# ZhangXinWhut/SimWhisper-Codec

Hardware: AMD Instinct MI355X
Metric: audio-sec/sec encode+decode (RTF^-1), 16kHz batch=32x10s (higher is better)
Workload: dtype split-f16 x3 encode (f32-class, f32 accumulate) / bf16 decode (f32 accumulate); 1 GPU; batch=32x10s @16kHz per GPU (32 utterances in all), encode()+decode(), 0.1*N(0,1) seed 1234, synthetic closed-form checkpoint (291M params); precision=mixed

## Files before the change

include/swc.h:

```cpp
#ifndef SWC_H_
#define SWC_H_

#include <stdint.h>

#ifdef __cplusplus
extern "C" {
#endif

#define SWC_OK 0
#define SWC_E_ARG (-1)
#define SWC_E_LAUNCH (-2)
#define SWC_E_NODEV (-3)

#define SWC_F32 0
#define SWC_BF16 1
#define SWC_F16S 2
#define SWC_F16S_ACT_SCALE 64.0f
#define SWC_FP8 3
#define SWC_FP8_ACT_SCALE 16.0f
#define SWC_F16 4

#define SWC_ACT_NONE 0
#define SWC_ACT_GELU 1

int swc_version(void);
const char* swc_last_error(void);
int swc_device_count(void);

int swc_delay_us(int32_t us, void* stream);

int swc_set_saturation_counter(uint32_t* counters);

typedef struct swc_gemm_args {
    const void* A;
    const void* W;
    void* C;
    const float* bias;
    const float* gamma;
    const float* residual;
    int64_t lda, ldw, ldc, ldr;
    int32_t M, N, K;
    int32_t taps, dil, stride, pad, t_in, t_out;
    int32_t a_dtype, c_dtype, act;
    float alpha;
    float out_scale;
} swc_gemm_args;
int swc_gemm(const swc_gemm_args* args, void* stream);
typedef struct swc_gemm_plan_out {
    int32_t a_dtype;
    int32_t tile_m, tile_n;
    int32_t waves;
    int32_t plain;
    int32_t act_body;
    int32_t k_slice, k_slices;
    int32_t n_tiles_m, n_tiles_n;
    int32_t band;
    int32_t grid, slots;
} swc_gemm_plan_out;
int swc_gemm_plan(const swc_gemm_args* args, swc_gemm_plan_out* plan);

int swc_attention(const void* qkv, void* out, const int32_t* lens, int32_t B, int32_t T,
                  int32_t H, int32_t dtype, void* stream);
int swc_attention16(const void* qkv, void* out, const int32_t* lens, int32_t B, int32_t T, int32_t H,
                    int32_t dtype, const int32_t* row_start, void* stream);
int swc_attention_ex(const void* qkv, void* out, const int32_t* lens, int32_t B, int32_t T, int32_t H,
                     int32_t out_dtype, void* stream);

int swc_layernorm(const float* x, void* y, const float* w, const float* b, const int32_t* lens,
                  int32_t B, int32_t t_in, int32_t t_out, int32_t C, float eps, int32_t y_dtype,
                  const int32_t* row_start, void* stream);

int swc_pack_rows(const void* src, void* dst, const int32_t* row_start, const int32_t* lens, int32_t B, int32_t T,
                  int64_t row_bytes, void* stream);

int64_t swc_convnext_stream_bytes(int32_t C, int32_t I);
int swc_convnext_pack(const void* w1_16bit, const void* w2_16bit, const float* gamma, void* w_stream, int32_t C, int32_t I,
                      void* stream);
int swc_convnext_mlp(const void* y, const void* w_stream, const float* b1, const float* b2, const float* gamma,
                     float* x, int32_t M, int32_t C, int32_t I, void* stream);
int swc_convnext_block(const float* x, float* x_out, const float* dw_w7, const float* dw_bias, const float* ln_w,
// ... 96 lines not shown
```

simwhisper_codec_amd/_lib.py:

```python
import ctypes as C
import os

import torch

HERE = os.path.dirname(os.path.abspath(__file__))
LIB_PATH = os.environ.get("SWC_LIB") or os.path.join(HERE, "libswc_hip.so")

F32, BF16, F16S, FP8 = 0, 1, 2, 3
F16S_ACT_SCALE = 64.0
FP8_ACT_SCALE = 16.0
ACT_NONE, ACT_GELU = 0, 1


class SwcError(RuntimeError):
    pass


class GemmArgs(C.Structure):
    _fields_ = [
        ("A", C.c_void_p), ("W", C.c_void_p), ("C", C.c_void_p),
        ("bias", C.c_void_p), ("gamma", C.c_void_p), ("residual", C.c_void_p),
        ("lda", C.c_int64), ("ldw", C.c_int64), ("ldc", C.c_int64), ("ldr", C.c_int64),
        ("M", C.c_int32), ("N", C.c_int32), ("K", C.c_int32),
        ("taps", C.c_int32), ("dil", C.c_int32), ("stride", C.c_int32), ("pad", C.c_int32),
        ("t_in", C.c_int32), ("t_out", C.c_int32),
        ("a_dtype", C.c_int32), ("c_dtype", C.c_int32), ("act", C.c_int32),
        ("alpha", C.c_float), ("out_scale", C.c_float),
    ]


class GemmPlan(C.Structure):
    _fields_ = [(n, C.c_int32) for n in ("a_dtype", "tile_m", "tile_n", "waves", "plain", "act_body", "k_slice", "k_slices",
                                         "n_tiles_m", "n_tiles_n", "band", "grid", "slots")]


class Dwconv7LnPlan(C.Structure):
    _fields_ = [(n, C.c_int32) for n in ("S", "NK", "FULL", "nst", "nstrips", "slots", "per", "grid")]


_P, _I, _L, _F = C.c_void_p, C.c_int32, C.c_int64, C.c_float

SIGNATURES = {
    "swc_gemm": [C.POINTER(GemmArgs), _P],
    "swc_gemm_plan": [C.POINTER(GemmArgs), C.POINTER(GemmPlan)],
    "swc_attention": [_P, _P, _P, _I, _I, _I, _I, _P],
    "swc_attention_ex": [_P, _P, _P, _I, _I, _I, _I, _P],
    "swc_attention16": [_P, _P, _P, _I, _I, _I, _I, _P, _P],
    "swc_layernorm": [_P, _P, _P, _P, _P, _I, _I, _I, _I, _F, _I, _P, _P],
    "swc_dwconv7_ln": [_P, _P, _P, _P, _P, _P, _I, _I, _I, _F, _I, _P],
    "swc_dwconv7_ln_plan": [_I, _I, _I, _I, C.POINTER(Dwconv7LnPlan)],
    "swc_snake_aa": [_P, _P, _P, _P, C.POINTER(_F), _I, _I, _I, _I, _P],
    "swc_fsq_encode": [_P, _L, _P, _P, _P, C.POINTER(_F), _I, _I, _I, _I, _P],
    "swc_fsq_decode": [_P, _P, _L, _P, _I, _I, _I, _P],
    "swc_fsq_encode_levels": [_P, _L, _P, _P, _P, C.POINTER(_F), C.POINTER(C.c_int32), _I, _I, _I, _I, _P],
    "swc_fsq_decode_levels": [_P, _P, _L, _P, C.POINTER(C.c_int32), _I, _I, _I, _P],
    "swc_mel_frames": [_P, _L, _P, _I, _P, _I, _I, _P],
# ... 90 lines not shown
```

simwhisper_codec_amd/codec.py:

```python
import functools
import logging
import math
import os
import threading

import torch
import torch.nn as nn
import yaml

from . import bitstream, ops, packed, spec, trace
from ._lib import SwcError

PRECISIONS = {"fp32": ("f32", "f32"), "mixed": ("f16s", "bf16"), "mixed_f32": ("f32", "bf16"), "bf16": ("bf16", "bf16"),
              "fp8": ("bf16", "bf16"), "fp8_fc1": ("bf16", "bf16"), "f16s": ("f16s", "f16s")}
_TORCH_DT = {"f32": torch.float32, "bf16": torch.bfloat16, "f16s": torch.float16}


_TLS = threading.local()


def _on_model_device(fn):
    @functools.wraps(fn)
    def wrapped(self, *a, **k):
        dev = self._buffers_device()
# ... 499 lines not shown
        else:
            P.c1w = W(conv_w(w1c), c1dt)
        P.c1b = V(sd["acoustic_encoder.conv1.bias"])
        P.c2w, P.c2b = W(conv_w(sd["acoustic_encoder.conv2.weight"]), edt), V(sd["acoustic_encoder.conv2.bias"])
        P.enc_ldt = ops.FP8_T if self._precision == "fp8" else edt
        P.enc_layers = layers("acoustic_encoder", e["encoder_layers"], P.enc_ldt,
                              fc1_dt=ops.FP8_T if self._precision == "fp8_fc1" else None)
        P.enc_ln = (V(sd["acoustic_encoder.layer_norm.weight"]), V(sd["acoustic_encoder.layer_norm.bias"]))
        ds = gp["downsample"]
        P.stack, P.hid, P.lat = ds["stack_factor"], ds["hidden_dim"], ds["latent_dim"]
        w = _fold_wn(sd, "downsample.in_proj")[:, :, 0]
        w = w.view(P.hid, ds["in_dim"], P.stack).permute(0, 2, 1).reshape(P.hid, -1)
        P.inw, P.inb = W(w, edt), V(sd["downsample.in_proj.bias"])
        P.down_units = res_units("downsample", edt)
        P.tlw, P.tlb = W(_fold_wn(sd, "downsample.to_latent")[:, :, 0], edt), V(sd["downsample.to_latent.bias"])
        q = gp["quantizer"]
        P.fsq = spec.fsq_constants(q["num_levels_per_group"], q.get("eps", 1e-3))

        us = gp["upsample"]
        P.uhid = us["hidden_dim"]
        P.udt = torch.float16 if (ddt == torch.bfloat16 and self.upsample_split_f16) else ddt
        P.flw, P.flb = W(_fold_wn(sd, "upsample.from_latent")[:, :, 0], P.udt), V(sd["upsample.from_latent.bias"])
        P.up_units = res_units("upsample", P.udt)
        w = _fold_wn(sd, "upsample.to_stacked")[:, :, 0]
        od = us["out_dim"]
        w = w.view(od, P.stack, -1).permute(1, 0, 2).reshape(od * P.stack, -1)
        b = sd["upsample.to_stacked.bias"].view(od, P.stack).T.reshape(-1)
        P.tsw, P.tsb = W(w, P.udt), V(b)
        dc = gp["acoustic_decoder"]
        P.Dd, P.Hd = dc["d_model"], dc["decoder_attention_heads"]
        P.dec_layers = layers("acoustic_decoder", dc["decoder_layers"], ddt)
        P.dec_ln = (V(sd["acoustic_decoder.layer_norm.weight"]), V(sd["acoustic_decoder.layer_norm.bias"]))
        P.io16 = ddt == torch.float16 or (ddt == torch.bfloat16 and self.decoder_io_split_f16 and dc["d_model"] % 32 == 0)
        iodt = torch.float16 if P.io16 else ddt
        w1 = sd["acoustic_decoder.deconv1.weight"]
        P.d1w, P.d1b = W(w1.permute(2, 1, 0).reshape(-1, w1.shape[0]), iodt), V(sd["acoustic_decoder.deconv1.bias"])
        w2 = sd["acoustic_decoder.deconv2.weight"]
        P.d2w = W(w2.flip(2).permute(1, 2, 0).reshape(w2.shape[1], -1), iodt)
        P.d2b = V(sd["acoustic_decoder.deconv2.bias"])
        v = gp["vocos"]
        P.vdim, P.vint, P.vin = v["dim"], v["intermediate_dim"], v["input_channels"]
        p = "vocos.backbone."
        dd16 = ddt == torch.float16
        P.vin_k = spec.cdiv(P.vin, 32) * 32 if P.io16 else P.vin
        P.tail16 = dd16 or (ddt == torch.bfloat16 and self.vocos_head_split_f16 and v["dim"] % 32 == 0)
        P.idft_k = 672 if P.tail16 else 648
# ... 93 lines not shown
        rounds = spec.cdiv(tiles, self.CUS)
        return tiles >= 0.6 * rounds * self.CUS

    convnext_f16 = False

    @staticmethod
    def _cx_f16_safe(sd, p, n_blocks, C):
        lim = 65504.0 / 8
        for i in range(n_blocks):
            b_ = f"{p}convnext.{i}."
            w1, w2 = sd[b_ + "pwconv1.weight"], sd[b_ + "pwconv2.weight"]
            if not (bool(torch.isfinite(w1).all()) and bool(torch.isfinite(w2).all())):
                return False
            if float(w1.abs().max()) >= lim or float(w2.abs().max()) >= lim:
                return False
            if math.sqrt(C) * float(sd[b_ + "norm.weight"].abs().max()) + float(sd[b_ + "norm.bias"].abs().max()) >= lim:
                return False
        return True

    layer_tail_f16 = True
    vocos_head_split_f16 = True
    decoder_io_split_f16 = False
    upsample_split_f16 = False
    conv1_split_f16 = True
    varlen_packing = True
    PACK_BELOW = 0.9

    def _pack_plan(self, lens_host, T, dt, dev):
        B = len(lens_host)
        total = sum(lens_host)
        if (not self.varlen_packing or dt == torch.float32 or total == 0 or total >= self.PACK_BELOW * B * T):
            return None, B * T
        cu, acc = [], 0
        for v in lens_host:
            cu.append(acc)
            acc += v
        return self._dev_ints(cu, dev), total

    def _res_units(self, h, units, B, T, C, dt):
        M = B * T
        for u in units:
            y = ops.snake_aa(h, u["a0"], u["b0"], u["f0"], B=B, T=T, C_=C, out_dtype=dt)
            y = self._mm(y, u["w1"], M, C, C, lda=C, ldw=7 * C, bias=u["c1"], taps=7, dil=u["dil"], pad=3 * u["dil"],
                         t_in=T, t_out=T)
            y = ops.snake_aa(y, u["a2"], u["b2"], u["f2"], B=B, T=T, C_=C, out_dtype=dt)
            self._mm(y, u["w3"], M, C, C, lda=C, bias=u["c3"], residual=h, out=h)
        return h

    def _logmel(self, wav, n_dev, n_host, P):
        with trace.stage("mel"):
            return self._logmel_impl(wav, n_dev, n_host, P)

    def _logmel_impl(self, wav, n_dev, n_host, P):
        B = wav.shape[0]
        Tm = min(spec.MEL_FRAMES, max(spec.mel_len(n) for n in n_host) + 2)
        fr = ops.mel_frames(wav, n_dev, spec.CHUNK_SAMPLES, B=B, T=Tm)
        M = B * Tm
        dft = self._mm(fr, P.dft, M, 402, 400, lda=400)
        pw = ops.mel_power(dft, 402, M, 208)
        mp = self._mm(pw, P.melw, M, P.n_mel, 208, lda=208)
        umax = torch.full((B,), -10.0 if Tm < spec.MEL_FRAMES else float("-inf"), device=wav.device, dtype=torch.float32)
        ops.mel_logmax(mp, P.n_mel, umax, B=B, T=Tm, n_mel=P.n_mel)
        mel = ops.mel_final(mp, P.n_mel, umax, B=B, T=Tm, n_mel=P.n_mel, ldo=P.c1k, out_dtype=P.c1dt)
        return mel, Tm

    def _encoder(self, mel, Tm, t_full, tok_host, P):
        with trace.stage("encoder"):
# ... 524 lines not shown
```

simwhisper_codec_amd/csrc/swc_api.hip:

```cpp
#include <stdarg.h>
#include "swc_common.h"

static thread_local char g_err[512] = "";

void swc_set_error(const char* fmt, ...) {
    va_list ap;
    va_start(ap, fmt);
    vsnprintf(g_err, sizeof(g_err), fmt, ap);
    va_end(ap);
}

static thread_local unsigned* g_sat = nullptr;
unsigned* swc_sat_counter() { return g_sat; }
extern "C" int swc_set_saturation_counter(uint32_t* dev_counters) {
    g_sat = dev_counters;
    return SWC_OK;
}

extern "C" int swc_version(void) { return 207; }

extern "C" const char* swc_last_error(void) { return g_err; }

extern "C" int swc_device_count(void) {
    int n = 0;
    hipError_t e = hipGetDeviceCount(&n);
    if (e != hipSuccess || n <= 0) {
        swc_set_error("swc_device_count: no HIP device (%s)", hipGetErrorString(e));
        return SWC_E_NODEV;
    }
    return n;
}
```

simwhisper_codec_amd/csrc/swc_gemm.hip:

```cpp
#include <string.h>
#include "swc_mfma.h"

static inline int tuning_env(const char* name, int dflt = 0) {
#ifdef SWC_TUNING
    const char* e = getenv(name);
    return e ? atoi(e) : dflt;
#else
    (void)name;
    return dflt;
#endif
}

namespace {


__device__ __attribute__((aligned(16))) unsigned int g_zero16[4] = {0u, 0u, 0u, 0u};
#ifdef SWC_GEMM_STAMP
__device__ unsigned long long g_stamps[512 * 8 * 8];
#endif


__device__ __forceinline__ int swz(int row) { return ((row >> 1) ^ ((row >> 4) << 1)) & 7; }
__device__ __forceinline__ int swz64(int row) { return ((-(row >> 2)) ^ (-(row >> 4))) & 3; }
template <int RB>
__device__ __forceinline__ int swz_rb(int row) { return RB == 128 ? swz(row) : swz64(row); }
template <int RB>
__device__ __forceinline__ int lds_off(int row, int chunk) { return row * RB + ((chunk ^ swz_rb<RB>(row)) << 4); }


struct GemmP {
    const char* A;
    const char* W;
    void* C;
    const float* bias;
    const float* gamma;
    const float* residual;
    long lda, ldw, ldc, ldr;
    int M, N, K;
    int taps, dil, stride, pad, t_in, t_out;
    int act;
    float alpha, out_scale;
    int band;
    unsigned* sat;
    int kc_per_tap;
    int n_tiles_n, n_tiles_m;
    int nt_mode;
    int stagger;
};

constexpr int EPI_TP = 68;
constexpr int EPI_WAVE_BYTES = 16 * EPI_TP * 4;


__device__ __forceinline__ void epi_st128(void* p, unsigned a, unsigned b, unsigned c, unsigned d, bool nt = false) {
#if defined(SWC_ABL_NOSTORE)
    asm volatile("" ::"v"(p), "v"(a), "v"(b), "v"(c), "v"(d));
#elif defined(SWC_EPI_PLAIN)
    (void)nt;
    *reinterpret_cast<uint4*>(p) = make_uint4(a, b, c, d);
#else
    if (nt) __builtin_nontemporal_store((u32x4){a, b, c, d}, reinterpret_cast<u32x4*>(p));
    else *reinterpret_cast<uint4*>(p) = make_uint4(a, b, c, d);
#endif
}
__device__ __forceinline__ void epi_st128f(void* p, float a, float b, float c, float d, bool nt = false) {
    epi_st128(p, __float_as_uint(a), __float_as_uint(b), __float_as_uint(c), __float_as_uint(d), nt);
}
__device__ __forceinline__ void epi_st64(void* p, unsigned a, unsigned b, bool nt = false) {
#if defined(SWC_ABL_NOSTORE)
    asm volatile("" ::"v"(p), "v"(a), "v"(b));
// ... 210 lines not shown
        const int colw = bn + wc * 64;
        const bool al16 = ((reinterpret_cast<uintptr_t>(p.C) | reinterpret_cast<uintptr_t>(p.residual) |
                            reinterpret_cast<uintptr_t>(p.bias) | reinterpret_cast<uintptr_t>(p.gamma)) & 15) == 0;
        const bool ok = tbuf && colw + 64 <= p.N && al16 && (p.ldc & (sizeof(OutT) == 1 ? 15 : 3)) == 0 &&
                        (!p.residual || (p.ldr & 3) == 0);
        if (__builtin_amdgcn_readfirstlane((int)ok)) {
            float amax = 0.f;
            if (gelu) gemm_epilogue_slab<OutT, MT, true>(p, acc, bm + wr * (MT * 16), colw, fr, fh, tbuf, amax, nt);
            else gemm_epilogue_slab<OutT, MT, false>(p, acc, bm + wr * (MT * 16), colw, fr, fh, tbuf, amax, nt);
            if constexpr (__is_same(OutT, fp8_t)) sat_commit(p.sat, 1, amax, SWC_FP8_LIMIT);
            return;
        }
    }
    if constexpr (ACT != 2) {
        gemm_epilogue_direct<OutT, MT, ACT>(p, acc, bm, bn, wr, wc, fr, fh, nt);
    } else if constexpr (__is_same(OutT, f16s_t) && MT == 8) {
        gemm_epilogue_direct<OutT, MT, 2>(p, acc, bm, bn, wr, wc, fr, fh, nt);
    } else {
        if (gelu) gemm_epilogue_direct<OutT, MT, 1>(p, acc, bm, bn, wr, wc, fr, fh, nt);
        else gemm_epilogue_direct<OutT, MT, 0>(p, acc, bm, bn, wr, wc, fr, fh, nt);
    }
}

template <int MODE, typename OutT, int MT, int WAVES_M, int WAVES_N, bool PLAIN, int RB = 128, int ACT = 2>
__global__ __launch_bounds__(WAVES_M* WAVES_N * 64, 2) void gemm_kernel(GemmP p) {
    constexpr int ROW_BYTES = RB;
    constexpr int CPR = RB / 16;
    constexpr int NG = RB / 64;
    static_assert(RB == 128 || (RB == 64 && MODE != SWC_F16S), "split-f16 needs hi|lo in one 128-byte row");
    static_assert(WAVES_M * WAVES_N * EPI_WAVE_BYTES <= (WAVES_M * MT * 16 + WAVES_N * 64) * RB, "epilogue scratch must fit one stage");
    constexpr bool BF16 = MODE == SWC_BF16;
    constexpr bool F16S = MODE == SWC_F16S;
    constexpr bool FP8 = MODE == SWC_FP8;
    constexpr int ES = BF16 ? 2 : (FP8 ? 1 : 4);
    constexpr int EPC = 16 / ES;
    constexpr int BK = ROW_BYTES / ES;
    constexpr int NT = WAVES_M * WAVES_N * 64;
    constexpr int BM = WAVES_M * MT * 16;
    constexpr int BN = WAVES_N * 64;
    constexpr int RPS = NT / CPR;
    constexpr int NA = BM / RPS;
    constexpr int NB = BN / RPS;
    constexpr int A_BYTES = BM * ROW_BYTES;
    constexpr int STAGE_BYTES = (BM + BN) * ROW_BYTES;

    extern __shared__ __attribute__((aligned(16))) char smem[];

    const int tid = threadIdx.x;
    const int lane = tid & 63;
    const int wave = tid >> 6;
    const int wr = wave / WAVES_N, wc = wave % WAVES_N;

    const int ntiles = p.n_tiles_m * p.n_tiles_n;
    const int xcd = blockIdx.x & 7;
    const int gw = ((int)gridDim.x - xcd + 7) >> 3;
    const int cq = ntiles >> 3, cr = ntiles & 7;
    const int chunk_start = xcd < cr ? xcd * (cq + 1) : cr * (cq + 1) + (xcd - cr) * cq;
    const int chunk_size = cq + (xcd < cr ? 1 : 0);
    int tl = blockIdx.x >> 3;
    if (tl >= chunk_size) return;
    int bm, bn;
    auto tile_origin = [&](int local) {
        const int bid = chunk_start + local;
        const int BAND = p.band;
        const int band = bid / (BAND * p.n_tiles_n);
        const int rem = bid - band * (BAND * p.n_tiles_n);
        const int rows_in_band = (p.n_tiles_m - band * BAND) < BAND ? (p.n_tiles_m - band * BAND) : BAND;
        const int tn = rem / rows_in_band;
        const int tm = band * BAND + (rem - tn * rows_in_band);
        bm = tm * BM;
        bn = tn * BN;
    };

    const int ld_pos = tid % CPR;
    const int ld_row = tid / CPR;
    int a_b[NA], a_t[NA], a_chunk[NA];
    bool a_rowok[NA];
    long w_rowoff[NB];
    int w_chunk[NB];
    bool w_rowok[NB];
    const int wave_u = __builtin_amdgcn_readfirstlane(wave);
    const unsigned smem_base = __builtin_amdgcn_readfirstlane(lds_addr_of(smem));
    constexpr int NV = RPS >= 64 ? 1 : 64 / RPS;
    unsigned chunkoff[NV];
#pragma unroll
    for (int v = 0; v < NV; ++v) chunkoff[v] = (unsigned)(ld_pos ^ swz_rb<RB>(ld_row + RPS * v)) << 4;
// ... 93 lines not shown
    auto dma_fence = [&]() {
        asm volatile("s_waitcnt lgkmcnt(0)" ::: "memory");
        const unsigned long long t1 = stamp();
        asm volatile("s_waitcnt vmcnt(0)" ::: "memory");
        const unsigned long long t2 = stamp();
        __syncthreads();
        const unsigned long long t3 = stamp();
        if (st_last) { st_cmp += t1 - st_last; st_vm += t2 - t1; st_bar += t3 - t2; st_n += 1; }
        st_last = t3;
    };
#else
    auto dma_fence = [&]() {
        asm volatile("s_waitcnt vmcnt(0)" ::: "memory");
        __syncthreads();
    };
#endif

    f32x4 acc[MT][4];
#pragma unroll
    for (int i = 0; i < MT; ++i)
#pragma unroll
        for (int j = 0; j < 4; ++j) acc[i][j] = (f32x4){0.f, 0.f, 0.f, 0.f};

    const int nkt = p.taps * p.kc_per_tap;
    const int fr = lane & 15, fh = lane >> 4;
    const int a_row0 = wr * (MT * 16) + fr;
    const int b_row0 = wc * 64 + 16 * (fr >> 2) + (fr & 3);
    stage_slice(0, 0);
    dma_fence();
#ifdef SWC_GEMM_PRIO47
    if (wave_u >= (WAVES_M * WAVES_N) / 2) __builtin_amdgcn_s_setprio(1);
#endif
    for (;;) {
    for (int kt = 0; kt < nkt; ++kt) {
        const int cur = kt & 1;
        if (kt + 1 < nkt) stage_slice(kt + 1, cur ^ 1);
#ifdef SWC_GEMM_IGLP
        __builtin_amdgcn_iglp_opt(SWC_GEMM_IGLP);
#endif
        const char* sa = smem + cur * STAGE_BYTES;
        const char* sb = sa + A_BYTES;
#ifdef SWC_GEMM_SPLIT
        constexpr bool EXPLICIT_SPLIT = (BF16 || F16S) && WAVES_M * WAVES_N == 8 && MT >= 4;
        constexpr int SPLIT = SWC_GEMM_SPLIT;
#else
        constexpr bool EXPLICIT_SPLIT = (F16S && WAVES_M * WAVES_N == 8 && MT >= 4) || ((BF16 || F16S) && WAVES_M * WAVES_N == 4);
        constexpr int SPLIT = WAVES_M * WAVES_N == 4 ? 0 : (MT == 8 ? 3 : 1);
#endif
        if constexpr (EXPLICIT_SPLIT) {
            uint4 f0a[MT], f0b[4], f1a[MT], f1b[4];
#pragma unroll
            for (int j = 0; j < 4; ++j) f0b[j] = *reinterpret_cast<const uint4*>(sb + lds_off<RB>(b_row0 + 4 * j, fh));
#pragma unroll
            for (int i = 0; i < MT; ++i) f0a[i] = *reinterpret_cast<const uint4*>(sa + lds_off<RB>(a_row0 + 16 * i, fh));
#pragma unroll
            for (int j = 0; j < 4; ++j) f1b[j] = *reinterpret_cast<const uint4*>(sb + lds_off<RB>(b_row0 + 4 * j, fh + 4));
#pragma unroll
            for (int i = 0; i < MT; ++i) f1a[i] = *reinterpret_cast<const uint4*>(sa + lds_off<RB>(a_row0 + 16 * i, fh + 4));
            auto mm = [&](int i) {
// ... 75 lines not shown
                            wa[4] = fb[j].x; wa[5] = fb[j].y; wa[6] = fb[j].z; wa[7] = fb[j].w;
                            xa[0] = ha[i].x; xa[1] = ha[i].y; xa[2] = ha[i].z; xa[3] = ha[i].w;
                            xa[4] = fa[i].x; xa[5] = fa[i].y; xa[6] = fa[i].z; xa[7] = fa[i].w;
                            acc[i][j] = __builtin_amdgcn_mfma_scale_f32_16x16x128_f8f6f4(wa, xa, acc[i][j], 0, 0, 0, 0x7f7f7f7f, 0,
                                                                                         0x7f7f7f7f);
                        }
                }
            } else {
#pragma unroll
                for (int e = 0; e < 4; ++e)
#pragma unroll
                    for (int i = 0; i < MT; ++i) {
                        const float av = __uint_as_float(reinterpret_cast<const unsigned*>(&fa[i])[e]);
#pragma unroll
                        for (int j = 0; j < 4; ++j) {
                            const float bv = __uint_as_float(reinterpret_cast<const unsigned*>(&fb[j])[e]);
                            acc[i][j] = __builtin_amdgcn_mfma_f32_16x16x4f32(bv, av, acc[i][j], 0, 0, 0);
                        }
                    }
            }
        }
        dma_fence();
    }
    const int bm_done = bm, bn_done = bn;
    tl += gw;
    const bool more = tl < chunk_size;
    if (more) {
        setup_tile(tl);
        stage_slice(0, 0);
    }
#ifdef SWC_GEMM_STAMP
    const unsigned long long st_e0 = stamp();
#endif
    gemm_epilogue<OutT, MT, MT < 8, ACT>(p, acc, bm_done, bn_done, wr, wc, fr, fh,
                            reinterpret_cast<float*>(smem + STAGE_BYTES + wave_u * EPI_WAVE_BYTES),
                            p.nt_mode == 2 || (p.nt_mode == 1 && !more));
#ifdef SWC_GEMM_STAMP
    asm volatile("s_waitcnt vmcnt(0)" ::: "memory");
    const unsigned long long st_e1 = stamp();
    if (lane == 0 && blockIdx.x < 512) {
        unsigned long long* o = g_stamps + ((long)blockIdx.x * 8 + wave) * 8;
        o[0] += st_cmp; o[1] += st_vm; o[2] += st_bar; o[3] += st_n; o[4] += st_e1 - st_e0; o[5] += 1; o[6] += st_e0 - st_last;
    }
    st_cmp = st_vm = st_bar = st_n = 0; st_last = 0;
#endif
    if (!more) break;
#pragma unroll
    for (int i = 0; i < MT; ++i)
#pragma unroll
        for (int j = 0; j < 4; ++j) acc[i][j] = (f32x4){0.f, 0.f, 0.f, 0.f};
    dma_fence();
    }
}

struct GemmPlan {
    int mode;
    int mt, wm, wn;
    int plain;
    int act_body;
    int bk;
    int kc_per_tap;
    int n_tiles_m, n_tiles_n;
    int band;
    long slots, grid;
    int nt_mode;
    int stagger;
};

template <int MODE, typename OutT, int MT, int WM, int WN, bool PLAIN, int RB = 128, int ACT = 2>
int launch_k(GemmP p, const GemmPlan& g, hipStream_t s) {
    constexpr int BM = WM * MT * 16, BN = WN * 64;
    constexpr int LDS = 2 * (BM + BN) * RB;
    constexpr int BK = RB / (MODE == SWC_BF16 ? 2 : (MODE == SWC_FP8 ? 1 : 4));
    if (g.mode != MODE || g.mt != MT || g.wm != WM || g.wn != WN || g.plain != (PLAIN ? 1 : 0) || g.act_body != ACT || g.bk != BK) {
        swc_set_error("swc_gemm: the launched kernel is not the planned one");
        return SWC_E_ARG;
    }
    p.kc_per_tap = g.kc_per_tap;
    p.n_tiles_n = g.n_tiles_n;
    p.n_tiles_m = g.n_tiles_m;
    p.band = g.band;
    p.nt_mode = g.nt_mode;
    p.stagger = g.stagger;
    auto kern = gemm_kernel<MODE, OutT, MT, WM, WN, PLAIN, RB, ACT>;
    if (LDS > 64 * 1024) SWC_ENABLE_LDS(kern, LDS, "swc_gemm");
    hipLaunchKernelGGL(kern, dim3((unsigned)g.grid), dim3(WM * WN * 64), LDS, s, p);
    return SWC_OK;
}

template <int MODE, typename OutT, int MT, int WM, int WN, int RB = 128>
int launch(GemmP p, const GemmPlan& g, hipStream_t s) {
    if constexpr (sizeof(OutT) < 4 && MODE != SWC_F32) {
        if (g.plain) return g.act_body == 1 ? launch_k<MODE, OutT, MT, WM, WN, true, RB, 1>(p, g, s) : launch_k<MODE, OutT, MT, WM, WN, true, RB, 0>(p, g, s);
        return launch_k<MODE, OutT, MT, WM, WN, false, RB, 2>(p, g, s);
    } else {
        return g.plain ? launch_k<MODE, OutT, MT, WM, WN, true, RB>(p, g, s) : launch_k<MODE, OutT, MT, WM, WN, false, RB>(p, g, s);
    }
}

int tile_override() { return tuning_env("SWC_GEMM_TILE"); }

int gemm_check_args(const swc_gemm_args* a) {
    SWC_CHECK_ARG(a != nullptr, "swc_gemm: null args");
    SWC_CHECK_ARG(a->A && a->W && a->C, "swc_gemm: null operand");
    SWC_CHECK_ARG(a->M >= 0 && a->N > 0 && a->K > 0, "swc_gemm: bad M/N/K %d %d %d", a->M, a->N, a->K);
    SWC_CHECK_ARG(a->a_dtype == SWC_F32 || a->a_dtype == SWC_BF16 || a->a_dtype == SWC_F16S || a->a_dtype == SWC_FP8,
                  "swc_gemm: bad a_dtype");
    SWC_CHECK_ARG(a->c_dtype == SWC_F32 || a->c_dtype == SWC_BF16 || a->c_dtype == SWC_F16S ||
                      (a->c_dtype == SWC_FP8 && a->a_dtype == SWC_FP8),
                  "swc_gemm: bad c_dtype (FP8 outputs come from FP8 operands only)");
    SWC_CHECK_ARG(a->c_dtype != SWC_F16S || a->a_dtype != SWC_FP8, "swc_gemm: fp8 operands have no split-f16 output");
    SWC_CHECK_ARG(a->c_dtype != SWC_F16S || a->a_dtype != SWC_BF16, "swc_gemm: bf16 operands have no split-f16 output");
    SWC_CHECK_ARG(a->c_dtype != SWC_BF16 || a->a_dtype != SWC_F16S, "swc_gemm: split-f16 operands have no bf16 output");
    SWC_CHECK_ARG(a->c_dtype != SWC_F16S || (a->N % 32 == 0 && a->ldc % 32 == 0 && aligned16(a->C)),
                  "swc_gemm: split-f16 output needs N, ldc multiples of 32 (N=%d)", a->N);
    SWC_CHECK_ARG(a->act == SWC_ACT_NONE || a->act == SWC_ACT_GELU, "swc_gemm: bad act");
    SWC_CHECK_ARG(!a->gamma || a->c_dtype == SWC_F32, "swc_gemm: gamma (per-column output scale) exists for f32 outputs only");
    const bool bf = a->a_dtype == SWC_BF16;
    const bool fs = a->a_dtype == SWC_F16S;
    const bool f8 = a->a_dtype == SWC_FP8;
    const int epc = bf ? 8 : (fs ? 32 : (f8 ? 16 : 4));
    SWC_CHECK_ARG(a->K % epc == 0, "swc_gemm: K=%d not a multiple of %d", a->K, epc);
    SWC_CHECK_ARG(a->lda % epc == 0 && a->ldw % epc == 0, "swc_gemm: lda/ldw break 16-byte rows");
    SWC_CHECK_ARG(aligned16(a->A) && aligned16(a->W), "swc_gemm: A/W not 16-byte aligned");
    SWC_CHECK_ARG(a->taps >= 1 && a->stride >= 1 && a->dil >= 1 && a->t_in >= 1 && a->t_out >= 1,
                  "swc_gemm: bad conv geometry");
    SWC_CHECK_ARG(a->M % a->t_out == 0, "swc_gemm: M=%d not a multiple of t_out=%d", a->M, a->t_out);
    SWC_CHECK_ARG(a->ldw >= (int64_t)a->taps * a->K, "swc_gemm: ldw < taps*K");
    SWC_CHECK_ARG(a->lda >= a->K && a->ldc >= a->N, "swc_gemm: lda < K or ldc < N");
    SWC_CHECK_ARG(!a->residual || a->ldr >= a->N, "swc_gemm: ldr < N");
    return SWC_OK;
}

int gemm_plan(const swc_gemm_args* a, GemmPlan* g) {
    const bool bf = a->a_dtype == SWC_BF16;
    const bool fs = a->a_dtype == SWC_F16S;
    const bool f8 = a->a_dtype == SWC_FP8;
    g->mode = a->a_dtype;
    const long big_tiles = (long)((a->M + 255) / 256) * ((a->N + 255) / 256);
    const bool fills = a->N >= 256 && big_tiles >= 96;
    bool big = (bf || f8 || fs) && fills;
    if (tile_override() == 128) big = false;
    if (tile_override() == 256) big = bf || f8 || fs;
    int mt = 8;
    if (big && (!fs || fills)) {
        const int forced = tuning_env("SWC_GEMM_MT");
        const long ntn = (a->N + 255) / 256;
        double best = 1e30;
        for (int cand : {8, 6, 4}) {
            const long tiles = ((a->M + cand * 32 - 1) / (cand * 32)) * ntn;
            const double cost = (double)((tiles + 255) / 256) * (cand + 1.5);
            if (cost < best - 1e-9) { best = cost; mt = cand; }
        }
// ... 14 lines not shown
                a->lda * es < (1L << 24) && a->ldw * es < (1L << 24))
                   ? 1 : 0;
    g->act_body = (a->c_dtype != SWC_F32 && a->a_dtype != SWC_F32 && g->plain) ? (a->act == SWC_ACT_GELU ? 1 : 0) : 2;
    g->kc_per_tap = (a->K + g->bk - 1) / g->bk;
    g->n_tiles_n = (a->N + BN - 1) / BN;
    g->n_tiles_m = (a->M + BM - 1) / BM;
    {
        const int forced = tuning_env("SWC_GEMM_BAND");
        g->band = forced > 0 ? forced : (g->n_tiles_n >= 12 ? 4 : 1);
    }
    const long nwg = (long)g->n_tiles_n * g->n_tiles_m;
    if (nwg >= (1L << 30)) {
        swc_set_error("swc_gemm: grid too large");
        return SWC_E_ARG;
    }
    const int persist = tuning_env("SWC_GEMM_NOPERSIST") ? 0 : 1;
    g->slots = 256L * (g->wm * g->wn == 4 ? 2 : 1);
    g->grid = (persist && nwg > g->slots) ? g->slots : nwg;
    g->nt_mode = tuning_env("SWC_GEMM_NT", 0);
    g->stagger = tuning_env("SWC_GEMM_STAGGER", 0);
    return SWC_OK;
}

}

extern "C" int swc_gemm_plan(const swc_gemm_args* a, swc_gemm_plan_out* out) {
    SWC_CHECK_ARG(out != nullptr, "swc_gemm_plan: null plan");
    memset(out, 0, sizeof(*out));
    int rc = gemm_check_args(a);
    if (rc != SWC_OK) return rc;
    if (a->M == 0) return SWC_OK;
    GemmPlan g;
    rc = gemm_plan(a, &g);
    if (rc != SWC_OK) return rc;
    out->a_dtype = g.mode;
    out->tile_m = g.wm * g.mt * 16;
    out->tile_n = g.wn * 64;
    out->waves = g.wm * g.wn;
    out->plain = g.plain;
    out->act_body = g.act_body;
    out->k_slice = g.bk;
    out->k_slices = g.kc_per_tap;
    out->n_tiles_m = g.n_tiles_m;
    out->n_tiles_n = g.n_tiles_n;
    out->band = g.band;
    out->grid = (int32_t)g.grid;
    out->slots = (int32_t)g.slots;
    return SWC_OK;
}

extern "C" int swc_gemm(const swc_gemm_args* a, void* stream) {
    int rc = gemm_check_args(a);
    if (rc != SWC_OK) return rc;
    if (a->M == 0) return SWC_OK;
    GemmPlan g;
    rc = gemm_plan(a, &g);
    if (rc != SWC_OK) return rc;

    GemmP p;
    p.A = (const char*)a->A;
    p.W = (const char*)a->W;
    p.C = a->C;
    p.bias = a->bias;
    p.gamma = a->gamma;
    p.residual = a->residual;
    p.lda = a->lda; p.ldw = a->ldw; p.ldc = a->ldc; p.ldr = a->ldr;
    p.M = a->M; p.N = a->N; p.K = a->K;
    p.taps = a->taps; p.dil = a->dil; p.stride = a->stride; p.pad = a->pad;
    p.t_in = a->t_in; p.t_out = a->t_out;
    p.act = a->act;
    p.alpha = a->alpha == 0.0f ? 1.0f : a->alpha;
    p.out_scale = a->out_scale == 0.0f ? 1.0f : a->out_scale;
    p.sat = swc_sat_counter();
    hipStream_t s = (hipStream_t)stream;
    const int cd = a->c_dtype;
    const int mt = g.mt;
    const bool big = g.wm * g.wn == 8;
#define SWC_LAUNCH(MODE, MT, WM, WN)                                                        \
    (cd == SWC_BF16 ? launch<MODE, bf16_t, MT, WM, WN>(p, g, s)                              \
                    : (cd == SWC_F16S ? launch<MODE, f16s_t, MT, WM, WN>(p, g, s) : launch<MODE, float, MT, WM, WN>(p, g, s)))
#define SWC_LAUNCH_B(MT, WM, WN) (cd == SWC_BF16 ? launch<SWC_BF16, bf16_t, MT, WM, WN>(p, g, s) : launch<SWC_BF16, float, MT, WM, WN>(p, g, s))
#define SWC_LAUNCH_S(MT, WM, WN) (cd == SWC_F16S ? launch<SWC_F16S, f16s_t, MT, WM, WN>(p, g, s) : launch<SWC_F16S, float, MT, WM, WN>(p, g, s))
    if (g.mode == SWC_FP8) {
#define SWC_LAUNCH8(MT, WM, WN)                                                   \
    (cd == SWC_BF16 ? launch<SWC_FP8, bf16_t, MT, WM, WN>(p, g, s)                  \
                    : (cd == SWC_FP8 ? launch<SWC_FP8, fp8_t, MT, WM, WN>(p, g, s) : launch<SWC_FP8, float, MT, WM, WN>(p, g, s)))
        if (big)
            rc = mt == 8 ? SWC_LAUNCH8(8, 2, 4) : (mt == 6 ? SWC_LAUNCH8(6, 2, 4) : SWC_LAUNCH8(4, 2, 4));
        else
            rc = SWC_LAUNCH8(4, 2, 2);
#undef SWC_LAUNCH8
    } else if (g.mode == SWC_BF16) {
        if (big)
            rc = mt == 8 ? SWC_LAUNCH_B(8, 2, 4) : (mt == 6 ? SWC_LAUNCH_B(6, 2, 4) : SWC_LAUNCH_B(4, 2, 4));
        else
            rc = mt == 2 ? SWC_LAUNCH_B(2, 2, 2) : SWC_LAUNCH_B(4, 2, 2);
    } else if (g.mode == SWC_F16S) {
        if (big)
            rc = mt == 8 ? SWC_LAUNCH_S(8, 2, 4) : (mt == 6 ? SWC_LAUNCH_S(6, 2, 4) : SWC_LAUNCH_S(4, 2, 4));
        else
            rc = mt == 2 ? SWC_LAUNCH_S(2, 2, 2) : SWC_LAUNCH_S(4, 2, 2);
    } else {
        rc = SWC_LAUNCH(SWC_F32, 4, 2, 2);
    }
#undef SWC_LAUNCH
#undef SWC_LAUNCH_B
// ... 18 lines not shown
```

simwhisper_codec_amd/ops.py:

```python
import ctypes as C

import torch

from . import _lib
from ._lib import ACT_GELU, ACT_NONE, BF16, F16S, F16S_ACT_SCALE, F32, FP8, FP8_ACT_SCALE

FP8_T = torch.float8_e4m3fn
_DT = {torch.float32: F32, torch.bfloat16: BF16, torch.float16: F16S, FP8_T: FP8}


def _w(dtype, cols):
    return 2 * cols if dtype == torch.float16 else cols

PROFILER = None
LEGACY_ATTENTION = False


def _stream():
    return C.c_void_p(torch._C._cuda_getCurrentRawStream(torch._C._cuda_getDevice()))


def _ptr(t):
    return C.c_void_p(t.data_ptr()) if t is not None else C.c_void_p(0)


def _chk(t, name, dtype=None):
    if not t.is_cuda:
        raise _lib.SwcError(f"{name}: expected a device tensor (the HIP path has no CPU fallback)")
    if t.device.index != torch._C._cuda_getDevice():
        raise _lib.SwcError(f"{name}: tensor on cuda:{t.device.index} but cuda:{torch._C._cuda_getDevice()} is current; kernels "
                            "run on the current device's stream (AudioCodec's entry points set it; direct ops callers "
                            "use torch.cuda.device)")
    if dtype is not None and t.dtype != dtype:
        raise _lib.SwcError(f"{name}: expected {dtype}, got {t.dtype}")
    return t


def _gemm_args(A, W, M, N, K, *, out=None, out_dtype=None, lda=None, ldw=None, ldc=None, bias=None, gamma=None,
               residual=None, ldr=None, act=ACT_NONE, taps=1, dil=1, stride=1, pad=0, t_in=None, t_out=None, alpha=1.0,
               out_scale=1.0):
    _chk(A, "gemm A"); _chk(W, "gemm W")
    if A.dtype != W.dtype:
        raise _lib.SwcError(f"gemm: A is {A.dtype} but W is {W.dtype}")
    sa = 2 if A.dtype == torch.float16 else 1
    lda = A.stride(-2) // sa if lda is None else lda
    ldw = W.stride(-2) // sa if ldw is None else ldw
    if out is None:
        od = out_dtype or torch.float32
        out = torch.empty((M, _w(od, N)), device=A.device, dtype=od)
    ldc = out.stride(-2) // (2 if out.dtype == torch.float16 else 1) if ldc is None else ldc
    a = _lib.GemmArgs()
    a.A, a.W, a.C = A.data_ptr(), W.data_ptr(), out.data_ptr()
    a.bias = bias.data_ptr() if bias is not None else None
    a.gamma = gamma.data_ptr() if gamma is not None else None
    a.residual = residual.data_ptr() if residual is not None else None
    a.lda, a.ldw, a.ldc = lda, ldw, ldc
    a.ldr = (residual.stride(-2) if ldr is None else ldr) if residual is not None else 0
    a.M, a.N, a.K = M, N, K
    a.taps, a.dil, a.stride, a.pad = taps, dil, stride, pad
    a.t_in = M if t_in is None else t_in
    a.t_out = M if t_out is None else t_out
    a.a_dtype, a.c_dtype, a.act = _DT[A.dtype], _DT[out.dtype], act
    a.alpha, a.out_scale = alpha, out_scale
    return a, out


def gemm(A, W, M, N, K, **kw):
    lib = _lib.load()
    a, out = _gemm_args(A, W, M, N, K, **kw)
    if M == 0:
        return out
    prof = PROFILER
    if prof is not None:
        prof.begin({torch.bfloat16: "gemm_bf16", torch.float16: "gemm_f16s", FP8_T: "gemm_fp8"}.get(A.dtype, "gemm_f32"),
                   2.0 * M * N * K * a.taps)
    _lib.check(lib.swc_gemm(C.byref(a), _stream()), "swc_gemm")
    if prof is not None:
        prof.end()
    return out


def gemm_call_plan(A, W, M, N, K, **kw):
    return gemm_plan(_gemm_args(A, W, M, N, K, **kw)[0])


def _plan_dict(st):
    return {name: int(getattr(st, name)) for name, _ in st._fields_}


def gemm_plan(args):
    out = _lib.GemmPlan()
    _lib.check(_lib.load().swc_gemm_plan(C.byref(args), C.byref(out)), "swc_gemm_plan")
    return _plan_dict(out)


def dwconv7_ln_plan(B, T, C_, out_dtype=torch.float32):
    out = _lib.Dwconv7LnPlan()
    _lib.check(_lib.load().swc_dwconv7_ln_plan(B, T, C_, _DT[out_dtype], C.byref(out)), "swc_dwconv7_ln_plan")
    return _plan_dict(out)


def attention(qkv, lens, B, T, H, out=None, out_dtype=None, row_start=None, rows=None):
# ... 540 lines not shown
```

Measured before the change: 15840 audio-s/s.

## Add split-K bf16 GEMM path with combine kernel for decoder upsample convs

```diff
diff --git a/include/swc.h b/include/swc.h
--- a/include/swc.h
+++ b/include/swc.h
@@ -44,7 +44,11 @@
     int32_t a_dtype, c_dtype, act;
     float alpha;
     float out_scale;
+    int32_t split_k;
+    void* workspace;
+    int64_t workspace_bytes;
 } swc_gemm_args;
+#define SWC_GEMM_MAX_SPLIT_K 16
 int swc_gemm(const swc_gemm_args* args, void* stream);
 typedef struct swc_gemm_plan_out {
     int32_t a_dtype;
@@ -56,6 +60,8 @@
     int32_t n_tiles_m, n_tiles_n;
     int32_t band;
     int32_t grid, slots;
+    int32_t k_split;
+    int64_t workspace_bytes;
 } swc_gemm_plan_out;
 int swc_gemm_plan(const swc_gemm_args* args, swc_gemm_plan_out* plan);
 
diff --git a/simwhisper_codec_amd/_lib.py b/simwhisper_codec_amd/_lib.py
--- a/simwhisper_codec_amd/_lib.py
+++ b/simwhisper_codec_amd/_lib.py
@@ -26,12 +26,13 @@
         ("t_in", C.c_int32), ("t_out", C.c_int32),
         ("a_dtype", C.c_int32), ("c_dtype", C.c_int32), ("act", C.c_int32),
         ("alpha", C.c_float), ("out_scale", C.c_float),
+        ("split_k", C.c_int32), ("workspace", C.c_void_p), ("workspace_bytes", C.c_int64),
     ]
 
 
 class GemmPlan(C.Structure):
     _fields_ = [(n, C.c_int32) for n in ("a_dtype", "tile_m", "tile_n", "waves", "plain", "act_body", "k_slice", "k_slices",
-                                         "n_tiles_m", "n_tiles_n", "band", "grid", "slots")]
+                                         "n_tiles_m", "n_tiles_n", "band", "grid", "slots", "k_split")] + [("workspace_bytes", C.c_int64)]
 
 
 class Dwconv7LnPlan(C.Structure):
diff --git a/simwhisper_codec_amd/codec.py b/simwhisper_codec_amd/codec.py
--- a/simwhisper_codec_amd/codec.py
+++ b/simwhisper_codec_amd/codec.py
@@ -545,6 +545,8 @@
         P.udt = torch.float16 if (ddt == torch.bfloat16 and self.upsample_split_f16) else ddt
         P.flw, P.flb = W(_fold_wn(sd, "upsample.from_latent")[:, :, 0], P.udt), V(sd["upsample.from_latent.bias"])
         P.up_units = res_units("upsample", P.udt)
+        for u in P.up_units:
+            u["ks"] = ops.split_k_factor(P.uhid, 7) if (self.decode_split_k and P.udt == torch.bfloat16) else 0
         w = _fold_wn(sd, "upsample.to_stacked")[:, :, 0]
         od = us["out_dim"]
         w = w.view(od, P.stack, -1).permute(1, 0, 2).reshape(od * P.stack, -1)
@@ -684,6 +686,7 @@
     vocos_head_split_f16 = True
     decoder_io_split_f16 = False
     upsample_split_f16 = False
+    decode_split_k = True
     conv1_split_f16 = True
     varlen_packing = True
     PACK_BELOW = 0.9
@@ -704,7 +707,7 @@
         for u in units:
             y = ops.snake_aa(h, u["a0"], u["b0"], u["f0"], B=B, T=T, C_=C, out_dtype=dt)
             y = self._mm(y, u["w1"], M, C, C, lda=C, ldw=7 * C, bias=u["c1"], taps=7, dil=u["dil"], pad=3 * u["dil"],
-                         t_in=T, t_out=T)
+                         t_in=T, t_out=T, split_k=u.get("ks", 0))
             y = ops.snake_aa(y, u["a2"], u["b2"], u["f2"], B=B, T=T, C_=C, out_dtype=dt)
             self._mm(y, u["w3"], M, C, C, lda=C, bias=u["c3"], residual=h, out=h)
         return h
diff --git a/simwhisper_codec_amd/csrc/swc_api.hip b/simwhisper_codec_amd/csrc/swc_api.hip
--- a/simwhisper_codec_amd/csrc/swc_api.hip
+++ b/simwhisper_codec_amd/csrc/swc_api.hip
@@ -17,7 +17,7 @@
     return SWC_OK;
 }
 
-extern "C" int swc_version(void) { return 207; }
+extern "C" int swc_version(void) { return 208; }
 
 extern "C" const char* swc_last_error(void) { return g_err; }
 
diff --git a/simwhisper_codec_amd/csrc/swc_gemm.hip b/simwhisper_codec_amd/csrc/swc_gemm.hip
--- a/simwhisper_codec_amd/csrc/swc_gemm.hip
+++ b/simwhisper_codec_amd/csrc/swc_gemm.hip
@@ -46,6 +46,8 @@
     int n_tiles_n, n_tiles_m;
     int nt_mode;
     int stagger;
+    int ksplit;
+    float* ws;
 };
 
 constexpr int EPI_TP = 68;
@@ -302,7 +304,7 @@
     }
 }
 
-template <int MODE, typename OutT, int MT, int WAVES_M, int WAVES_N, bool PLAIN, int RB = 128, int ACT = 2>
+template <int MODE, typename OutT, int MT, int WAVES_M, int WAVES_N, bool PLAIN, int RB = 128, int ACT = 2, int KS = 0>
 __global__ __launch_bounds__(WAVES_M* WAVES_N * 64, 2) void gemm_kernel(GemmP p) {
     constexpr int ROW_BYTES = RB;
     constexpr int CPR = RB / 16;
@@ -331,7 +333,7 @@
     const int wave = tid >> 6;
     const int wr = wave / WAVES_N, wc = wave % WAVES_N;
 
-    const int ntiles = p.n_tiles_m * p.n_tiles_n;
+    const int ntiles = p.n_tiles_m * p.n_tiles_n * (KS ? p.ksplit : 1);
     const int xcd = blockIdx.x & 7;
     const int gw = ((int)gridDim.x - xcd + 7) >> 3;
     const int cq = ntiles >> 3, cr = ntiles & 7;
@@ -340,8 +342,17 @@
     int tl = blockIdx.x >> 3;
     if (tl >= chunk_size) return;
     int bm, bn;
+    const int nkt = p.taps * p.kc_per_tap;
+    int kslice = 0, kt0 = 0, ktn = nkt;
     auto tile_origin = [&](int local) {
-        const int bid = chunk_start + local;
+        int bid = chunk_start + local;
+        if constexpr (KS) {
+            const int per = p.n_tiles_m * p.n_tiles_n;
+            kslice = bid / per;
+            bid -= kslice * per;
+            kt0 = (int)((long)kslice * nkt / p.ksplit);
+            ktn = (int)((long)(kslice + 1) * nkt / p.ksplit) - kt0;
+        }
         const int BAND = p.band;
         const int band = bid / (BAND * p.n_tiles_n);
         const int rem = bid - band * (BAND * p.n_tiles_n);
@@ -481,19 +492,18 @@
 #pragma unroll
         for (int j = 0; j < 4; ++j) acc[i][j] = (f32x4){0.f, 0.f, 0.f, 0.f};
 
-    const int nkt = p.taps * p.kc_per_tap;
     const int fr = lane & 15, fh = lane >> 4;
     const int a_row0 = wr * (MT * 16) + fr;
     const int b_row0 = wc * 64 + 16 * (fr >> 2) + (fr & 3);
-    stage_slice(0, 0);
+    stage_slice(kt0, 0);
     dma_fence();
 #ifdef SWC_GEMM_PRIO47
     if (wave_u >= (WAVES_M * WAVES_N) / 2) __builtin_amdgcn_s_setprio(1);
 #endif
     for (;;) {
-    for (int kt = 0; kt < nkt; ++kt) {
+    for (int kt = 0; kt < ktn; ++kt) {
         const int cur = kt & 1;
-        if (kt + 1 < nkt) stage_slice(kt + 1, cur ^ 1);
+        if (kt + 1 < ktn) stage_slice(kt0 + kt + 1, cur ^ 1);
 #ifdef SWC_GEMM_IGLP
         __builtin_amdgcn_iglp_opt(SWC_GEMM_IGLP);
 #endif
@@ -615,19 +625,29 @@
         }
         dma_fence();
     }
-    const int bm_done = bm, bn_done = bn;
+    const int bm_done = bm, bn_done = bn, kslice_done = kslice;
     tl += gw;
     const bool more = tl < chunk_size;
     if (more) {
         setup_tile(tl);
-        stage_slice(0, 0);
+        stage_slice(kt0, 0);
     }
 #ifdef SWC_GEMM_STAMP
     const unsigned long long st_e0 = stamp();
 #endif
+    if constexpr (KS) {
+        GemmP q = p;
+        q.C = p.ws + (long)kslice_done * p.M * p.N;
+        q.ldc = p.N;
+        q.bias = nullptr; q.gamma = nullptr; q.residual = nullptr;
+        q.alpha = 1.0f;
+        gemm_epilogue<float, MT, MT < 8, 0>(q, acc, bm_done, bn_done, wr, wc, fr, fh,
+                                reinterpret_cast<float*>(smem + STAGE_BYTES + wave_u * EPI_WAVE_BYTES), false);
+    } else {
     gemm_epilogue<OutT, MT, MT < 8, ACT>(p, acc, bm_done, bn_done, wr, wc, fr, fh,
                             reinterpret_cast<float*>(smem + STAGE_BYTES + wave_u * EPI_WAVE_BYTES),
                             p.nt_mode == 2 || (p.nt_mode == 1 && !more));
+    }
 #ifdef SWC_GEMM_STAMP
     asm volatile("s_waitcnt vmcnt(0)" ::: "memory");
     const unsigned long long st_e1 = stamp();
@@ -643,6 +663,61 @@
 #pragma unroll
         for (int j = 0; j < 4; ++j) acc[i][j] = (f32x4){0.f, 0.f, 0.f, 0.f};
     dma_fence();
+    }
+}
+
+template <typename OutT>
+__global__ __launch_bounds__(256) void gemm_splitk_combine(GemmP p) {
+    const int n4 = (p.N + 3) >> 2;
+    const long idx = (long)blockIdx.x * 256 + threadIdx.x;
+    if (idx >= (long)p.M * n4) return;
+    const int row = (int)(idx / n4);
+    const int col = (int)(idx - (long)row * n4) * 4;
+    const long slice = (long)p.M * p.N;
+    const float* w = p.ws + (long)row * p.N + col;
+    const bool gelu = p.act == SWC_ACT_GELU;
+    OutT* C = reinterpret_cast<OutT*>(p.C) + (long)row * p.ldc + col;
+    const float* res = p.residual ? p.residual + (long)row * p.ldr + col : nullptr;
+    constexpr int OA = sizeof(OutT) == 4 ? 15 : 7;
+    const bool vec = col + 4 <= p.N && (p.N & 3) == 0 && (p.ldc & 3) == 0 && (reinterpret_cast<uintptr_t>(p.C) & OA) == 0 &&
+                     (!res || ((p.ldr & 3) == 0 && (reinterpret_cast<uintptr_t>(p.residual) & 15) == 0));
+    float v[4];
+    if (vec) {
+        float4 a = *reinterpret_cast<const float4*>(w);
+        for (int s = 1; s < p.ksplit; ++s) {
+            const float4 b = *reinterpret_cast<const float4*>(w + s * slice);
+            a.x += b.x; a.y += b.y; a.z += b.z; a.w += b.w;
+        }
+        v[0] = a.x; v[1] = a.y; v[2] = a.z; v[3] = a.w;
+    } else {
+#pragma unroll
+        for (int c = 0; c < 4; ++c) {
+            v[c] = 0.f;
+            if (col + c >= p.N) continue;
+            v[c] = w[c];
+            for (int s = 1; s < p.ksplit; ++s) v[c] += w[s * slice + c];
+        }
+    }
+#pragma unroll
+    for (int c = 0; c < 4; ++c) {
+        if (col + c >= p.N) continue;
+        float x = v[c] * p.alpha + (p.bias ? p.bias[col + c] : 0.f);
+        if (gelu) x = epi_act<OutT>(x);
+        if (p.gamma) x *= p.gamma[col + c];
+        if (res && !vec) x += res[c];
+        v[c] = x;
+    }
+    if (vec) {
+        if (res) {
+            const float4 r = *reinterpret_cast<const float4*>(res);
+            v[0] += r.x; v[1] += r.y; v[2] += r.z; v[3] += r.w;
+        }
+        if constexpr (sizeof(OutT) == 4) epi_st128f(C, v[0], v[1], v[2], v[3]);
+        else epi_st64(C, bf16_pack2(v[0], v[1]), bf16_pack2(v[2], v[3]));
+    } else {
+#pragma unroll
+        for (int c = 0; c < 4; ++c)
+            if (col + c < p.N) store_out<OutT>(C + c, v[c]);
     }
 }
 
@@ -658,14 +733,16 @@
     long slots, grid;
     int nt_mode;
     int stagger;
+    int ksplit;
 };
 
-template <int MODE, typename OutT, int MT, int WM, int WN, bool PLAIN, int RB = 128, int ACT = 2>
+template <int MODE, typename OutT, int MT, int WM, int WN, bool PLAIN, int RB = 128, int ACT = 2, int KS = 0>
 int launch_k(GemmP p, const GemmPlan& g, hipStream_t s) {
     constexpr int BM = WM * MT * 16, BN = WN * 64;
     constexpr int LDS = 2 * (BM + BN) * RB;
     constexpr int BK = RB / (MODE == SWC_BF16 ? 2 : (MODE == SWC_FP8 ? 1 : 4));
-    if (g.mode != MODE || g.mt != MT || g.wm != WM || g.wn != WN || g.plain != (PLAIN ? 1 : 0) || g.act_body != ACT || g.bk != BK) {
+    if (g.mode != MODE || g.mt != MT || g.wm != WM || g.wn != WN || g.plain != (PLAIN ? 1 : 0) || g.act_body != ACT || g.bk != BK ||
+        (g.ksplit > 1) != (KS != 0)) {
         swc_set_error("swc_gemm: the launched kernel is not the planned one");
         return SWC_E_ARG;
     }
@@ -675,7 +752,8 @@
     p.band = g.band;
     p.nt_mode = g.nt_mode;
     p.stagger = g.stagger;
-    auto kern = gemm_kernel<MODE, OutT, MT, WM, WN, PLAIN, RB, ACT>;
+    p.ksplit = g.ksplit;
+    auto kern = gemm_kernel<MODE, OutT, MT, WM, WN, PLAIN, RB, ACT, KS>;
     if (LDS > 64 * 1024) SWC_ENABLE_LDS(kern, LDS, "swc_gemm");
     hipLaunchKernelGGL(kern, dim3((unsigned)g.grid), dim3(WM * WN * 64), LDS, s, p);
     return SWC_OK;
@@ -689,6 +767,19 @@
     } else {
         return g.plain ? launch_k<MODE, OutT, MT, WM, WN, true, RB>(p, g, s) : launch_k<MODE, OutT, MT, WM, WN, false, RB>(p, g, s);
     }
+}
+
+template <int MT, int WM, int WN>
+int launch_splitk(GemmP p, const GemmPlan& g, int c_dtype, hipStream_t s) {
+    const int rc = g.plain ? launch_k<SWC_BF16, float, MT, WM, WN, true, 128, 2, 1>(p, g, s)
+                           : launch_k<SWC_BF16, float, MT, WM, WN, false, 128, 2, 1>(p, g, s);
+    if (rc != SWC_OK) return rc;
+    p.ksplit = g.ksplit;
+    const long threads = (long)p.M * ((p.N + 3) / 4);
+    const dim3 grid((unsigned)((threads + 255) / 256));
+    if (c_dtype == SWC_BF16) hipLaunchKernelGGL(gemm_splitk_combine<bf16_t>, grid, dim3(256), 0, s, p);
+    else hipLaunchKernelGGL(gemm_splitk_combine<float>, grid, dim3(256), 0, s, p);
+    return SWC_OK;
 }
 
 int tile_override() { return tuning_env("SWC_GEMM_TILE"); }
@@ -722,6 +813,10 @@
     SWC_CHECK_ARG(a->ldw >= (int64_t)a->taps * a->K, "swc_gemm: ldw < taps*K");
     SWC_CHECK_ARG(a->lda >= a->K && a->ldc >= a->N, "swc_gemm: lda < K or ldc < N");
     SWC_CHECK_ARG(!a->residual || a->ldr >= a->N, "swc_gemm: ldr < N");
+    SWC_CHECK_ARG(a->split_k >= 0 && a->split_k <= SWC_GEMM_MAX_SPLIT_K, "swc_gemm: split_k=%d outside [0, %d]", a->split_k,
+                  SWC_GEMM_MAX_SPLIT_K);
+    SWC_CHECK_ARG(a->split_k <= 1 || (a->a_dtype == SWC_BF16 && (a->c_dtype == SWC_F32 || a->c_dtype == SWC_BF16)),
+                  "swc_gemm: split_k exists for bf16 operands with f32 / bf16 outputs only");
     return SWC_OK;
 }
 
@@ -782,6 +877,48 @@
     return SWC_OK;
 }
 
+int gemm_plan_splitk(const swc_gemm_args* a, GemmPlan* g) {
+    g->mode = SWC_BF16;
+    g->bk = 64;
+    g->kc_per_tap = (a->K + g->bk - 1) / g->bk;
+    const long steps = (long)a->taps * g->kc_per_tap;
+    g->ksplit = (int)(a->split_k < steps ? a->split_k : steps);
+    g->mt = 4; g->wm = 2; g->wn = 2;
+    const int t = tuning_env("SWC_SPLITK_TILE");
+    if (t == 64) g->mt = 2;
+    if (t == 256) g->wn = 4;
+    const int BM = g->wm * g->mt * 16, BN = g->wn * 64;
+    g->plain = ((a->taps == 1) && (a->K % g->bk == 0) && (a->stride == 1) && (a->pad == 0) && (a->t_in == a->t_out) &&
+                a->lda * 2 < (1L << 24) && a->ldw * 2 < (1L << 24)) ? 1 : 0;
+    g->act_body = 2;
+    g->n_tiles_n = (a->N + BN - 1) / BN;
+    g->n_tiles_m = (a->M + BM - 1) / BM;
+    g->band = g->n_tiles_n >= 12 ? 4 : 1;
+    const long nwg = (long)g->n_tiles_n * g->n_tiles_m * g->ksplit;
+    if (nwg >= (1L << 30)) {
+        swc_set_error("swc_gemm: grid too large");
+        return SWC_E_ARG;
+    }
+    g->slots = 256L * (g->wm * g->wn == 4 ? 2 : 1);
+    g->grid = nwg > g->slots ? g->slots : nwg;
+    g->nt_mode = 0;
+    g->stagger = 0;
+    return SWC_OK;
+}
+
+int gemm_plan_any(const swc_gemm_args* a, GemmPlan* g) {
+    if (a->split_k > 1) {
+        const int rc = gemm_plan_splitk(a, g);
+        if (rc != SWC_OK || g->ksplit > 1) return rc;
+    }
+    g->ksplit = 1;
+    return gemm_plan(a, g);
+}
+
+long splitk_workspace_bytes(const swc_gemm_args* a, const GemmPlan& g) {
+    return g.ksplit > 1 ? (long)g.ksplit * a->M * a->N * 4 : 0;
+}
+
 }
 
 extern "C" int swc_gemm_plan(const swc_gemm_args* a, swc_gemm_plan_out* out) {
@@ -791,7 +928,7 @@
     if (rc != SWC_OK) return rc;
     if (a->M == 0) return SWC_OK;
     GemmPlan g;
-    rc = gemm_plan(a, &g);
+    rc = gemm_plan_any(a, &g);
     if (rc != SWC_OK) return rc;
     out->a_dtype = g.mode;
     out->tile_m = g.wm * g.mt * 16;
@@ -806,6 +943,8 @@
     out->band = g.band;
     out->grid = (int32_t)g.grid;
     out->slots = (int32_t)g.slots;
+    out->k_split = g.ksplit;
+    out->workspace_bytes = splitk_workspace_bytes(a, g);
     return SWC_OK;
 }
 
@@ -814,8 +953,13 @@
     if (rc != SWC_OK) return rc;
     if (a->M == 0) return SWC_OK;
     GemmPlan g;
-    rc = gemm_plan(a, &g);
+    rc = gemm_plan_any(a, &g);
     if (rc != SWC_OK) return rc;
+    if (g.ksplit > 1) {
+        SWC_CHECK_ARG(a->workspace && aligned16(a->workspace) && a->workspace_bytes >= splitk_workspace_bytes(a, g),
+                      "swc_gemm: split_k=%d needs a 16-byte aligned workspace of %ld bytes (swc_gemm_plan reports it), got %ld",
+                      a->split_k, splitk_workspace_bytes(a, g), (long)a->workspace_bytes);
+    }
 
     GemmP p;
     p.A = (const char*)a->A;
@@ -832,6 +976,8 @@
     p.alpha = a->alpha == 0.0f ? 1.0f : a->alpha;
     p.out_scale = a->out_scale == 0.0f ? 1.0f : a->out_scale;
     p.sat = swc_sat_counter();
+    p.ksplit = g.ksplit;
+    p.ws = g.ksplit > 1 ? (float*)a->workspace : nullptr;
     hipStream_t s = (hipStream_t)stream;
     const int cd = a->c_dtype;
     const int mt = g.mt;
@@ -841,7 +987,9 @@
                     : (cd == SWC_F16S ? launch<MODE, f16s_t, MT, WM, WN>(p, g, s) : launch<MODE, float, MT, WM, WN>(p, g, s)))
 #define SWC_LAUNCH_B(MT, WM, WN) (cd == SWC_BF16 ? launch<SWC_BF16, bf16_t, MT, WM, WN>(p, g, s) : launch<SWC_BF16, float, MT, WM, WN>(p, g, s))
 #define SWC_LAUNCH_S(MT, WM, WN) (cd == SWC_F16S ? launch<SWC_F16S, f16s_t, MT, WM, WN>(p, g, s) : launch<SWC_F16S, float, MT, WM, WN>(p, g, s))
-    if (g.mode == SWC_FP8) {
+    if (g.ksplit > 1) {
+        rc = big ? launch_splitk<4, 2, 4>(p, g, cd, s) : (mt == 2 ? launch_splitk<2, 2, 2>(p, g, cd, s) : launch_splitk<4, 2, 2>(p, g, cd, s));
+    } else if (g.mode == SWC_FP8) {
 #define SWC_LAUNCH8(MT, WM, WN)                                                   \
     (cd == SWC_BF16 ? launch<SWC_FP8, bf16_t, MT, WM, WN>(p, g, s)                  \
                     : (cd == SWC_FP8 ? launch<SWC_FP8, fp8_t, MT, WM, WN>(p, g, s) : launch<SWC_FP8, float, MT, WM, WN>(p, g, s)))
diff --git a/simwhisper_codec_amd/ops.py b/simwhisper_codec_amd/ops.py
--- a/simwhisper_codec_amd/ops.py
+++ b/simwhisper_codec_amd/ops.py
@@ -38,7 +38,7 @@
 
 def _gemm_args(A, W, M, N, K, *, out=None, out_dtype=None, lda=None, ldw=None, ldc=None, bias=None, gamma=None,
                residual=None, ldr=None, act=ACT_NONE, taps=1, dil=1, stride=1, pad=0, t_in=None, t_out=None, alpha=1.0,
-               out_scale=1.0):
+               out_scale=1.0, split_k=0, workspace=None):
     _chk(A, "gemm A"); _chk(W, "gemm W")
     if A.dtype != W.dtype:
         raise _lib.SwcError(f"gemm: A is {A.dtype} but W is {W.dtype}")
@@ -62,6 +62,10 @@
     a.t_out = M if t_out is None else t_out
     a.a_dtype, a.c_dtype, a.act = _DT[A.dtype], _DT[out.dtype], act
     a.alpha, a.out_scale = alpha, out_scale
+    a.split_k = split_k
+    if workspace is not None:
+        _chk(workspace, "gemm workspace")
+        a.workspace, a.workspace_bytes = workspace.data_ptr(), workspace.numel() * workspace.element_size()
     return a, out
 
 
@@ -70,6 +74,9 @@
     a, out = _gemm_args(A, W, M, N, K, **kw)
     if M == 0:
         return out
+    if a.split_k > 1 and not a.workspace:
+        ws = torch.empty(a.split_k * M * N, device=A.device, dtype=torch.float32)
+        a.workspace, a.workspace_bytes = ws.data_ptr(), ws.numel() * 4
     prof = PROFILER
     if prof is not None:
         prof.begin({torch.bfloat16: "gemm_bf16", torch.float16: "gemm_f16s", FP8_T: "gemm_fp8"}.get(A.dtype, "gemm_f32"),
@@ -78,6 +85,14 @@
     if prof is not None:
         prof.end()
     return out
+
+
+SPLIT_K_MIN = 2048
+SPLIT_K = 4
+
+
+def split_k_factor(K, taps=1):
+    return SPLIT_K if taps * K >= SPLIT_K_MIN else 0
 
 
 def gemm_call_plan(A, W, M, N, K, **kw):
```

Result: no change. 15900 audio-s/s, median of 6 (+0.4%).
